# FlagArihant2000/sfm-mvs

Hardware: AMD Instinct MI355X
Metric: descriptor-pair distances/sec (BF-KNN k=2 + Lowe ratio) (higher is better)
Workload: dtype f32 results (bit-identical to the direct-form f32 reference); filter arithmetic on MFMA: i8 MFMA on the descriptors QUANTISED to 8 bits (one grid per pair; the certificate uses the measured residua...; 1 GPU; BASELINE configs[1]: 10k x 10k uniform[0,1) float32 128-D descriptors, BF-KNN k=2 + Lowe ratio 0.70; a step = one launch set = a batch of 8 distinct pairs of that shape per GPU (8e8 distances; 8 distinct pairs per launch set, 2 sets of images rotating over the steps); nq=10000, nt=10000, dim=128

## Files before the change

sfm_mvs_amd/csrc/knn.hip:

```cpp
#include "common.h"
#include <cfloat>
#include <climits>
#include <cstdlib>
#include <type_traits>
#include <algorithm>
#include <mutex>
#include <vector>

namespace {

typedef float f32x16 __attribute__((ext_vector_type(16)));
typedef float f32x4 __attribute__((ext_vector_type(4)));
typedef float f32x3 __attribute__((ext_vector_type(3), aligned(4)));
typedef int i32x3 __attribute__((ext_vector_type(3), aligned(4)));

constexpr int kDim = 128;
constexpr int kTileT = 32;


constexpr int kResidentWaves = 4096;
constexpr int kMaxSlots = 258;
constexpr float kInf = __builtin_huge_valf();
constexpr int kSubTilesHost = 64;
constexpr int kI8SubTilesHost = 128;
// ... 1560 lines not shown
#pragma unroll
        for (int g = 0; g < 2; ++g)
            if (qok[g]) {
                const int64_t ob = ((int64_t)(qrow0 + 32 * g) * (2 * smax * nsub) + (int64_t)slot * nsub * 2 + h) * 3;
                for (int e = sub + 1; e < nsub; ++e)
#pragma unroll
                    for (int r = 0; r < 3; ++r) {
                        cand_s[ob + 6 * e + r] = kInf;
                        cand_i[ob + 6 * e + r] = -1;
                    }
            }
        wait_vmcnt<0>();
        u += t_end - t_begin;
    }
}

template <int ABL, int W>
__global__ __launch_bounds__(64 * W, 2) void knn_filter_split2_kernel(
    const unsigned short* __restrict__ qsplit, const float* __restrict__ qnorm, int nq, int nq_pad,
    const unsigned short* __restrict__ tsplit, int nt, int nt_pad, const float* __restrict__ tn, int tiles, int64_t units,
    int smax, int nsub, const int* __restrict__ midflag, const float* __restrict__ bmax, int force_mode,
    float* __restrict__ cand_s, int* __restrict__ cand_i, const int64_t* __restrict__ wg_begin, const int* __restrict__ rb_first,
    int n_rb1, int n_pairs, int64_t s_qsplit, int64_t s_tsplit, int64_t s_qn, int64_t s_tn, int64_t s_cand, int* __restrict__ minfo,
    const float* __restrict__ bmaxerr, long long* __restrict__ trace) {
    extern __shared__ __attribute__((aligned(16))) float smem[];
    if (trace && threadIdx.x == 0) {
        trace[4 * blockIdx.x + 0] = wall_clock64();
        trace[4 * blockIdx.x + 2] = __builtin_amdgcn_s_getreg(0xF804);
        trace[4 * blockIdx.x + 3] = __builtin_amdgcn_s_getreg(0xF814);
        trace[8192 + 4 * blockIdx.x + 2] = clock64();
    }
    const bool need_mid = (force_mode >= 0 ? force_mode : minfo[kMinfoBatchMode]) == kModeSplit;
    if (need_mid)
        filter_split2_body<ABL, W, true>(smem, qsplit, qnorm, nq, nq_pad, tsplit, nt_pad, tn, tiles, units, smax, nsub, cand_s, cand_i, wg_begin, rb_first,
                                         n_rb1, s_qsplit, s_tsplit, s_qn, s_tn, s_cand, trace);
    else
        filter_split2_body<ABL, W, false>(smem, qsplit, qnorm, nq, nq_pad, tsplit, nt_pad, tn, tiles, units, smax, nsub, cand_s, cand_i, wg_begin, rb_first,
                                          n_rb1, s_qsplit, s_tsplit, s_qn, s_tn, s_cand, trace);
    if (trace && threadIdx.x == 0) {
        trace[4 * blockIdx.x + 1] = wall_clock64();
        trace[8192 + 4 * blockIdx.x + 3] = clock64();
    }
}

constexpr int kQ4Rows = 4 * 4 * 32;
constexpr int kQ4Ring = 3;

typedef int i32x4 __attribute__((ext_vector_type(4)));
typedef int i32x2 __attribute__((ext_vector_type(2)));
typedef unsigned u32x2 __attribute__((ext_vector_type(2)));
#define SFM_MFMA_F16(acc, a, b) asm volatile("v_mfma_f32_32x32x16_f16 %0, %1, %2, %0" : "+v"(acc) : "v"(a), "a"(b))
#define SFM_MFMA_BF16(acc, a, b) asm volatile("v_mfma_f32_32x32x16_bf16 %0, %1, %2, %0" : "+v"(acc) : "v"(a), "a"(b))
#define SFM_MFMA_BF16_INIT(acc, a, b) asm volatile("v_mfma_f32_32x32x8_bf16 %0, %1, %2, 0" : "=v"(acc) : "v"(a), "a"(b))
#define SFM_MFMA_BF16_REINIT(acc, a, b) asm volatile("v_mfma_f32_32x32x8_bf16 %0, %1, %2, 0" : "+v"(acc) : "v"(a), "a"(b))
#define SFM_MFMA_F16_C(acc, a, b, c) asm volatile("v_mfma_f32_32x32x16_f16 %0, %1, %2, %3" : "=&v"(acc) : "v"(a), "a"(b), "v"(c))
#define SFM_MFMA_BF16_C(acc, a, b, c) asm volatile("v_mfma_f32_32x32x16_bf16 %0, %1, %2, %3" : "=&v"(acc) : "v"(a), "a"(b), "v"(c))

__device__ __forceinline__ void key_insert_quad(const f32x16& a, int r, int seq , int vmask, int& k0, int& k1, int& k2) {
    const int m = min(min(__float_as_int(a[r]), __float_as_int(a[r + 1])), min(__float_as_int(a[r + 2]), __float_as_int(a[r + 3])));
    int key;
    asm("v_and_or_b32 %0, %1, %2, %3" : "=v"(key) : "v"(m), "v"(vmask), "s"(seq));
    const int lo = min(key, k0);
    const int m1 = max(min(key, k1), min(max(key, k1), k0));
    k2 = max(min(key, k1), min(max(key, k1), k2));
    k1 = m1;
    k0 = lo;
}

__device__ __forceinline__ int key_make(const f32x16& a, int r, int seq , int vmask) {
    const int m = min(min(__float_as_int(a[r]), __float_as_int(a[r + 1])), min(__float_as_int(a[r + 2]), __float_as_int(a[r + 3])));
    int key;
    asm("v_and_or_b32 %0, %1, %2, %3" : "=v"(key) : "v"(m), "v"(vmask), "s"(seq));
    return key;
}
__device__ __forceinline__ void key_put(int key, int& k0, int& k1, int& k2) {
    const int lo = min(key, k0);
    const int m1 = max(min(key, k1), min(max(key, k1), k0));
    k2 = max(min(key, k1), min(max(key, k1), k2));
    k1 = m1;
    k0 = lo;
}

template <bool KMID, int ABL>
__device__ __forceinline__ void filter_q4_body(
    const unsigned char* __restrict__ qfrag, const unsigned char* __restrict__ tfrag, const unsigned char* __restrict__ qhm,
    const unsigned char* __restrict__ thm, int nq, int nq_pad, int tiles, int smax, int nsub, float* __restrict__ cand_s0,
    int* __restrict__ cand_i0, const int64_t* __restrict__ wg_begin, const int* __restrict__ rb_first, int n_rb1, int64_t s_qfrag,
    int64_t s_tfrag, int64_t s_qhm, int64_t s_thm, int64_t s_cand, const int* __restrict__ minfo, const int* __restrict__ wg_sbase) {
    constexpr int NG = KMID ? 2 : 4;
    constexpr int NPASS = KMID ? 2 : 1;
    constexpr int P = NG / 2;
    constexpr int D = KMID ? 2 : kQ4Ring;
    constexpr int NF = KMID ? 16 : 8;
    const int lane = threadIdx.x & 63;
    const int wave = __builtin_amdgcn_readfirstlane(threadIdx.x >> 6);
    const int j = lane & 31, h = lane >> 5;
    const int G = gridDim.x;
    const int bid = (G & 7) == 0 ? (int)(blockIdx.x & 7) * (G >> 3) + (int)(blockIdx.x >> 3) : (int)blockIdx.x;
    const int64_t u_end = wg_begin[bid + 1];
    int64_t u = wg_begin[bid];
    const int voff = lane * 16, voffi = lane * 8;
    const int qtiles = nq_pad >> 5;
    int vmask;
    asm volatile("v_mov_b32 %0, %1" : "=v"(vmask) : "s"(~kKeyMask));

    while (u < u_end) {
        const int rb = __builtin_amdgcn_readfirstlane((int)(u / tiles));
        const int t_begin = __builtin_amdgcn_readfirstlane((int)(u - (int64_t)rb * tiles));
        const int t_end = __builtin_amdgcn_readfirstlane((int)min((int64_t)tiles, t_begin + (u_end - u)));
        const int sbase = __builtin_amdgcn_readfirstlane(u == wg_begin[bid] ? wg_sbase[bid] : 0);
        const int pb = __builtin_amdgcn_readfirstlane(n_rb1 > 0 ? rb / n_rb1 : 0);
        const int rbl = rb - pb * n_rb1;
        float* __restrict__ cand_s = cand_s0 + pb * s_cand;
        int* __restrict__ cand_i = cand_i0 + pb * s_cand;
        const __amdgpu_buffer_rsrc_t trs = __builtin_amdgcn_make_buffer_rsrc((void*)(tfrag + pb * s_tfrag), 0, tiles * kTileFragBytes, 0x00020000);
        const __amdgpu_buffer_rsrc_t qrs = __builtin_amdgcn_make_buffer_rsrc((void*)(qfrag + pb * s_qfrag), 0, qtiles * kTileFragBytes, 0x00020000);
        const __amdgpu_buffer_rsrc_t thrs = __builtin_amdgcn_make_buffer_rsrc((void*)(KMID ? thm + pb * s_thm : tfrag), 0, KMID ? tiles * 16 * kFragBytes : 0, 0x00020000);
        const __amdgpu_buffer_rsrc_t qhrs = __builtin_amdgcn_make_buffer_rsrc((void*)(KMID ? qhm + pb * s_qhm : qfrag), 0, KMID ? qtiles * 16 * kFragBytes : 0, 0x00020000);

#pragma unroll 1
        for (int pass = 0; pass < NPASS; ++pass) {
            const int qg0 = rbl * (kQ4Rows / 32) + wave * 4 + pass * NG;
            const int qrow0 = qg0 * 32 + j;
            bool qok[NG];
#pragma unroll
            for (int g = 0; g < NG; ++g) qok[g] = qrow0 + 32 * g < nq;

            i32x4 fr[D][NF];
            i32x2 fri[D];
            auto load_frag = [&](int s, int f, int tile_, bool live, bool in_loop = false) {
                if ((ABL & 1) && in_loop) return;
                const int tile = (ABL & 4) ? t_begin : live ? tile_ : t_end - 1;
                if (f == NF) {
                    fri[s] = __builtin_amdgcn_raw_buffer_load_b64(trs, voffi, __builtin_amdgcn_readfirstlane(tile * kTileFragBytes + 8 * kFragBytes), 0);
                } else if constexpr (KMID) {
                    fr[s][f] = __builtin_amdgcn_raw_buffer_load_b128(thrs, voff, __builtin_amdgcn_readfirstlane(tile * (16 * kFragBytes) + f * kFragBytes), 0);
                } else {
                    fr[s][f] = __builtin_amdgcn_raw_buffer_load_b128(trs, voff, __builtin_amdgcn_readfirstlane(tile * kTileFragBytes + f * kFragBytes), 0);
                }
            };
#pragma unroll
            for (int d = 0; d < D; ++d) {
                load_frag(d, NF, t_begin + d, t_begin + d < t_end);
#pragma unroll
                for (int f = 0; f < NF; ++f) load_frag(d, f, t_begin + d, t_begin + d < t_end);
            }

            __builtin_amdgcn_sched_barrier(0);
            u32x4 bq[NG][KMID ? 16 : 8];
            u32x2 bi;
            {
                i32x4 tmp[NG][KMID ? 16 : 8];
#pragma unroll
                for (int g = 0; g < NG; ++g) {
#pragma unroll
                    for (int f = 0; f < (KMID ? 16 : 8); ++f)
                        tmp[g][f] = KMID ? __builtin_amdgcn_raw_buffer_load_b128(qhrs, voff, __builtin_amdgcn_readfirstlane((qg0 + g) * (16 * kFragBytes) + f * kFragBytes), 0)
                                         : __builtin_amdgcn_raw_buffer_load_b128(qrs, voff, __builtin_amdgcn_readfirstlane((qg0 + g) * kTileFragBytes + f * kFragBytes), 0);
                }
                const uint2 qm = frag_init_operand(__int_as_float(minfo[kMinfoQmax + pb]), true, h);
                __builtin_amdgcn_sched_barrier(0);
#pragma unroll
                for (int g = 0; g < NG; ++g) {
#pragma unroll
                    for (int f = 0; f < (KMID ? 16 : 8); ++f) asm volatile("" : "=a"(bq[g][f]) : "0"(__builtin_bit_cast(u32x4, tmp[g][f])));
                }
                asm volatile("" : "=a"(bi) : "0"(u32x2{qm.x, qm.y}));
            }
            asm volatile("s_nop 4");

            int k0[NG], k1[NG], k2[NG];
#pragma unroll
            for (int g = 0; g < NG; ++g) k0[g] = k1[g] = k2[g] = kKeyInf;
            int sub = 0, sub_t0 = t_begin;
            auto flush = [&](int sb, int st0) {
                int qr = qrow0;
                asm volatile("" : "+v"(qr));
#pragma unroll
                for (int g = 0; g < NG; ++g) {
                    if (qok[g]) {
                        const int64_t ob = ((int64_t)(qr + 32 * g) * (2 * smax * nsub) + (int64_t)(sbase + sb) * 2 + h) * 3;
                        flush_keys<true>(k0[g], k1[g], k2[g], st0, h, cand_s + ob, cand_i + ob);
                    }
                    k0[g] = k1[g] = k2[g] = kKeyInf;
                }
            };
            f32x16 acc[NG];
#pragma unroll
            for (int g = P; g < NG; ++g)
#pragma unroll
                for (int r = 0; r < 16; ++r) acc[g][r] = kInf;
            f32x16 cinit;
            SFM_MFMA_BF16_INIT(cinit, __builtin_bit_cast(u32x2, fri[0]), bi);
            asm volatile("s_nop 15\n\ts_nop 7" ::: "memory");

            auto tile = [&](int t, auto slot_c) {
                constexpr int S = decltype(slot_c)::value;
                const bool more = t + D < t_end;
                const int seq_prev = __builtin_amdgcn_readfirstlane(max((t - 1) - sub_t0, 0) << 2);
#pragma unroll
                for (int st = 0; st < 8; ++st) {
                    __builtin_amdgcn_sched_barrier(0);
                    const u32x4 a = __builtin_bit_cast(u32x4, fr[S][st]);
                    if constexpr (KMID) {
                        const u32x4 am = __builtin_bit_cast(u32x4, fr[S][8 + st]);
                        if (st == 0) SFM_MFMA_BF16_C(acc[0], a, bq[0][st], cinit);
                        else SFM_MFMA_BF16(acc[0], a, bq[0][st]);
                        SFM_MFMA_BF16(acc[0], a, bq[0][8 + st]);
                        SFM_MFMA_BF16(acc[0], am, bq[0][st]);
                        if (st & 1) key_insert_quad(acc[1], 4 * (st >> 1), seq_prev + (st >> 1), vmask, k0[1], k1[1], k2[1]);
                    } else {
                        const int g = 2 + (st >> 2);
                        if (st == 0) SFM_MFMA_F16_C(acc[0], a, bq[0][st], cinit);
                        else SFM_MFMA_F16(acc[0], a, bq[0][st]);
                        int key = 0;
                        if (!(ABL & 2)) key = key_make(acc[g], 4 * (st & 3), seq_prev + (st & 3), vmask);
                        __builtin_amdgcn_sched_barrier(0);
                        if (st == 0) SFM_MFMA_F16_C(acc[1], a, bq[1][st], cinit);
                        else SFM_MFMA_F16(acc[1], a, bq[1][st]);
                        if (ABL & 2) {
                            if (st == 0) k0[2] = min(k0[2], __float_as_int(acc[2][0]) + __float_as_int(acc[3][5]));
                        } else
                            key_put(key, k0[g], k1[g], k2[g]);
                    }
                    __builtin_amdgcn_sched_barrier(0);
                }
                if (t - sub_t0 == kSubTiles) {
                    flush(sub, sub_t0);
                    ++sub;
                    sub_t0 = t;
                }
                const int seq_cur = __builtin_amdgcn_readfirstlane((t - sub_t0) << 2);
                __builtin_amdgcn_sched_barrier(0);
                load_frag(S, NF, t + D, more, true);
#pragma unroll
                for (int st = 0; st < 8; ++st) {
                    __builtin_amdgcn_sched_barrier(0);
                    const u32x4 a = __builtin_bit_cast(u32x4, fr[S][st]);
                    if constexpr (KMID) {
                        const u32x4 am = __builtin_bit_cast(u32x4, fr[S][8 + st]);
                        if (st == 0) SFM_MFMA_BF16_C(acc[1], a, bq[1][st], cinit);
                        else SFM_MFMA_BF16(acc[1], a, bq[1][st]);
                        SFM_MFMA_BF16(acc[1], a, bq[1][8 + st]);
                        SFM_MFMA_BF16(acc[1], am, bq[1][st]);
                        if (st == 1) SFM_MFMA_BF16_REINIT(cinit, __builtin_bit_cast(u32x2, fri[(S + 1) % D]), bi);
                    } else {
                        const int g = st >> 2;
                        if (st == 0) SFM_MFMA_F16_C(acc[2], a, bq[2][st], cinit);
                        else SFM_MFMA_F16(acc[2], a, bq[2][st]);
                        int key = 0;
                        if (!(ABL & 2)) key = key_make(acc[g], 4 * (st & 3), seq_cur + (st & 3), vmask);
                        __builtin_amdgcn_sched_barrier(0);
                        if (st == 0) SFM_MFMA_F16_C(acc[3], a, bq[3][st], cinit);
                        else SFM_MFMA_F16(acc[3], a, bq[3][st]);
                        if (st == 1) SFM_MFMA_BF16_REINIT(cinit, __builtin_bit_cast(u32x2, fri[(S + 1) % D]), bi);
                        __builtin_amdgcn_sched_barrier(0);
                        load_frag(S, st, t + D, more, true);
                        if (ABL & 2) {
                            if (st == 0) k0[0] = min(k0[0], __float_as_int(acc[0][0]) + __float_as_int(acc[1][5]));
                        } else
                            key_put(key, k0[g], k1[g], k2[g]);
                    }
                    if constexpr (KMID) {
                        __builtin_amdgcn_sched_barrier(0);
                        load_frag(S, st, t + D, more, true);
                        load_frag(S, 8 + st, t + D, more, true);
                        if (st & 1) key_insert_quad(acc[0], 4 * (st >> 1), seq_cur + (st >> 1), vmask, k0[0], k1[0], k2[0]);
                    }
                    __builtin_amdgcn_sched_barrier(0);
                }
            };
            int t = t_begin;
            for (; t + D <= t_end; t += D) {
                tile(t, std::integral_constant<int, 0>{});
                tile(t + 1, std::integral_constant<int, 1>{});
                if constexpr (D > 2) tile(t + 2, std::integral_constant<int, (D > 2 ? 2 : 0)>{});
            }
            if (t < t_end) {
                tile(t, std::integral_constant<int, 0>{});
                if constexpr (D > 2)
                    if (t + 1 < t_end) tile(t + 1, std::integral_constant<int, 1>{});
            }
            asm volatile("s_nop 15\n\ts_nop 15" ::: "memory");
            if (t_end > t_begin) {
                const int seq = __builtin_amdgcn_readfirstlane(((t_end - 1) - sub_t0) << 2);
#pragma unroll
                for (int g = P; g < NG; ++g)
#pragma unroll
                    for (int r = 0; r < 16; r += 4) key_insert_quad(acc[g], r, seq + (r >> 2), vmask, k0[g], k1[g], k2[g]);
            }
            flush(sub, sub_t0);
        }
        u += t_end - t_begin;
    }
}


typedef int i32x16 __attribute__((ext_vector_type(16)));
#define SFM_MFMA_I8(acc, a, b) asm volatile("v_mfma_i32_32x32x32_i8 %0, %1, %2, %0" : "+v"(acc) : "v"(a), "a"(b))
#define SFM_MFMA_I8_C(acc, a, b, c) asm volatile("v_mfma_i32_32x32x32_i8 %0, %1, %2, %3" : "=&v"(acc) : "v"(a), "a"(b), "v"(c))
#define SFM_MFMA_I8_INIT(acc, a, b) asm volatile("v_mfma_i32_32x32x32_i8 %0, %1, %2, 0" : "=v"(acc) : "v"(a), "a"(b))
#define SFM_MFMA_I8_REINIT(acc, a, b) asm volatile("v_mfma_i32_32x32x32_i8 %0, %1, %2, 0" : "+v"(acc) : "v"(a), "a"(b))

__device__ __forceinline__ int key_pack_i8(int m, int seq ) {
    int key;
    asm("v_lshl_or_b32 %0, %1, 8, %2" : "=v"(key) : "v"(m), "s"(seq));
    return key;
}
__device__ __forceinline__ int imin3(int a, int b, int c) { return min(min(a, b), c); }

template <int ABL>
__device__ __forceinline__ void filter_i8_body(
    const unsigned char* __restrict__ qi8, const unsigned char* __restrict__ ti8, int nq, int nq_pad, int nt, int tiles, int nstr ,
    int* __restrict__ keys0, int* __restrict__ sttab0, const int64_t* __restrict__ wg_begin, int n_rb1, int64_t s_qi8, int64_t s_ti8, int64_t s_keys,
    const int* __restrict__ wg_sbase, int G, int sub_tiles ) {
    constexpr int NG = kI8Groups, P = NG / 2, D = 2;
    const int lane = threadIdx.x & 63;
    const int wave = __builtin_amdgcn_readfirstlane(threadIdx.x >> 6);
    const int j = lane & 31, h = lane >> 5;
    const int bid = (G & 7) == 0 ? (int)(blockIdx.x & 7) * (G >> 3) + (int)(blockIdx.x >> 3) : (int)blockIdx.x;
    const int64_t u_end = wg_begin[bid + 1];
    int64_t u = wg_begin[bid];
    auto train_off = [](int l) { return ((l & ~12) | ((l & 4) << 1) | ((l & 8) >> 1)) * 16; };
    const int voff_t = train_off(lane);
    const int qtiles = nq_pad >> 5;

    while (u < u_end) {
        const int rb = __builtin_amdgcn_readfirstlane((int)(u / tiles));
        const int t_begin = __builtin_amdgcn_readfirstlane((int)(u - (int64_t)rb * tiles));
        const int t_end = __builtin_amdgcn_readfirstlane((int)min((int64_t)tiles, t_begin + (u_end - u)));
        const int sbase = __builtin_amdgcn_readfirstlane(u == wg_begin[bid] ? wg_sbase[bid] : 0);
        const int pb = __builtin_amdgcn_readfirstlane(n_rb1 > 0 ? rb / n_rb1 : 0);
        const int rbl = rb - pb * n_rb1;
        int* __restrict__ keys = keys0 + pb * s_keys;
        int* __restrict__ sttab = sttab0 + (int64_t)rb * nstr * 2;
        const __amdgpu_buffer_rsrc_t trs = __builtin_amdgcn_make_buffer_rsrc((void*)(ti8 + pb * s_ti8), 0, tiles * kI8TileBytes, 0x00020000);
        const __amdgpu_buffer_rsrc_t qrs = __builtin_amdgcn_make_buffer_rsrc((void*)(qi8 + pb * s_qi8), 0, qtiles * kI8QTileBytes, 0x00020000);
        const int qg0 = rbl * (kI8Rows / 32) + wave * NG;
        const int qloc0 = wave * NG * 32 + j;

        i32x4 fr[D][5];
        auto load_frag = [&](int s_, int f, int tile_, bool live, bool in_loop = false) {
            if ((ABL & 1) && in_loop) return;
            const int tile = live ? tile_ : t_end - 1;
            fr[s_][f] = __builtin_amdgcn_raw_buffer_load_b128(trs, voff_t, __builtin_amdgcn_readfirstlane(tile * kI8TileBytes + f * 1024), 0);
        };
#pragma unroll
        for (int d = 0; d < D; ++d) {
            load_frag(d, 4, t_begin + d, t_begin + d < t_end);
#pragma unroll
            for (int f = 0; f < 4; ++f) load_frag(d, f, t_begin + d, t_begin + d < t_end);
        }
        __builtin_amdgcn_sched_barrier(0);
        u32x4 bq[NG][4], bi;
        {
            i32x4 tmp[NG][4];
            int voff_q = voff_t;
            asm volatile("" : "+v"(voff_q));
            const int sw = (voff_q ^ (voff_q >> 1)) & 64;
            voff_q ^= sw | (sw << 1);
#pragma unroll
            for (int g = 0; g < NG; ++g)
#pragma unroll
                for (int f = 0; f < 4; ++f)
                    tmp[g][f] = __builtin_amdgcn_raw_buffer_load_b128(qrs, voff_q, __builtin_amdgcn_readfirstlane((qg0 + g) * kI8QTileBytes + f * 1024), 0);
            __builtin_amdgcn_sched_barrier(0);
#pragma unroll
            for (int g = 0; g < NG; ++g)
#pragma unroll
                for (int f = 0; f < 4; ++f) asm volatile("" : "=a"(bq[g][f]) : "0"(__builtin_bit_cast(u32x4, tmp[g][f])));
            asm volatile("" : "=a"(bi) : "0"(u32x4{h ? 0x80808080u : 0x80808001u, 0x80808080u, 0x80808080u, 0x80808080u}));
        }
        asm volatile("s_nop 4");

        int k0[NG], k1[NG], k2[NG];
#pragma unroll
        for (int g = 0; g < NG; ++g) k0[g] = k1[g] = k2[g] = INT_MAX;
        int sub = 0, sub_t0 = t_begin;
        auto flush = [&](int sb, int st0, int st1) {
            int vo = qloc0 * 16 + h * (kI8Rows * 16);
            asm volatile("" : "+v"(vo));
            const __amdgpu_buffer_rsrc_t krs = __builtin_amdgcn_make_buffer_rsrc(
                (void*)(keys + (int64_t)(rbl * nstr + sbase + sb) * (2 * kI8Rows * 4)), 0, 2 * kI8Rows * 16, 0x00020000);
#pragma unroll
            for (int g = 0; g < NG; ++g) {
                __builtin_amdgcn_raw_buffer_store_b128(u32x4{(unsigned)k0[g], (unsigned)k1[g], (unsigned)k2[g], (unsigned)INT_MAX}, krs, vo + 512 * g, 0, 0);
                k0[g] = k1[g] = k2[g] = INT_MAX;
            }
            if (threadIdx.x == 0) {
                sttab[2 * (sbase + sb)] = st0;
                sttab[2 * (sbase + sb) + 1] = st1 - st0;
            }
        };
        i32x16 acc[NG], cinit;
#pragma unroll
        for (int g = P; g < NG; ++g)
#pragma unroll
            for (int r = 0; r < 16; ++r) acc[g][r] = 0x7FFFFF;
        SFM_MFMA_I8_INIT(cinit, __builtin_bit_cast(u32x4, fr[0][4]), bi);
        asm volatile("s_nop 15\n\ts_nop 7" ::: "memory");

        const int nrem = nt & 31;
        auto mask_tail = [&](i32x16& a) {
#pragma unroll
            for (int r = 0; r < 16; ++r) a[r] = 16 * (r >> 3) + 8 * h + (r & 7) >= nrem ? 0x7FFFFF : a[r];
        };
        int m0 = 0, m1 = 0, n0 = 0, n1 = 0, key = 0, key2 = 0;
        auto epi = [&](int piece, i32x16& a, int seq , int& e0, int& e1, int& e2, bool partial) {
            if (ABL & 2) { if (piece == 0) e0 = min(e0, a[0] + a[15]); return; }
            if (piece == 0 && partial) mask_tail(a);
            if (piece == 0) { m0 = imin3(a[0], a[1], a[2]); n0 = imin3(a[8], a[9], a[10]); m1 = imin3(a[3], a[4], a[5]); n1 = imin3(a[11], a[12], a[13]); }
            else if (piece == 1) { m0 = imin3(m0, m1, a[6]); n0 = imin3(n0, n1, a[14]); m0 = min(m0, a[7]); n0 = min(n0, a[15]); }
            else if (piece == 2) { key = key_pack_i8(m0, seq); key2 = key_pack_i8(n0, seq | 1); key_put(key, e0, e1, e2); }
            else key_put(key2, e0, e1, e2);
            if (piece >= 2) asm volatile("" : "+v"(e0), "+v"(e1), "+v"(e2));
        };
        auto tile = [&](int t, auto slot_c, auto flush_c) {
            constexpr int S = decltype(slot_c)::value;
            constexpr int FL = decltype(flush_c)::value;
            const bool more = t + D < t_end;
            const int seq_prev = __builtin_amdgcn_readfirstlane(max((t - 1) - sub_t0, 0) << 1);
            const bool part_cur = nrem != 0 && t + 1 == tiles;
#pragma unroll
            for (int st = 0; st < 4; ++st) {
                const u32x4 a = __builtin_bit_cast(u32x4, fr[S][st]);
#pragma unroll
                for (int g = 0; g < P; ++g) {
                    __builtin_amdgcn_sched_barrier(0);
                    if (st == 0) SFM_MFMA_I8_C(acc[g], a, bq[g][st], cinit);
                    else SFM_MFMA_I8(acc[g], a, bq[g][st]);
                    epi(g, acc[P + st], seq_prev, k0[P + st], k1[P + st], k2[P + st], false);
                    __builtin_amdgcn_sched_barrier(0);
                }
            }
            if (FL == 1 || (FL == 2 && t - sub_t0 == sub_tiles)) {
                flush(sub, sub_t0, t);
                ++sub;
                sub_t0 = t;
            }
            const int seq_cur = __builtin_amdgcn_readfirstlane((t - sub_t0) << 1);
            __builtin_amdgcn_sched_barrier(0);
            load_frag(S, 4, t + D, more, true);
#pragma unroll
            for (int st = 0; st < 4; ++st) {
                const u32x4 a = __builtin_bit_cast(u32x4, fr[S][st]);
#pragma unroll
                for (int g = 0; g < P; ++g) {
                    __builtin_amdgcn_sched_barrier(0);
                    if (st == 0) SFM_MFMA_I8_C(acc[P + g], a, bq[P + g][st], cinit);
                    else SFM_MFMA_I8(acc[P + g], a, bq[P + g][st]);
                    if (st == 1 && g == 1) SFM_MFMA_I8_REINIT(cinit, __builtin_bit_cast(u32x4, fr[(S + 1) % D][4]), bi);
                    epi(g, acc[st], seq_cur, k0[st], k1[st], k2[st], part_cur);
                    __builtin_amdgcn_sched_barrier(0);
                }
                load_frag(S, st, t + D, more, true);
            }
        };
        constexpr std::integral_constant<int, 0> c0{};
        constexpr std::integral_constant<int, 1> c1{};
        constexpr std::integral_constant<int, 2> c2{};
        int t = t_begin;
        for (;;) {
            const int t_stop = __builtin_amdgcn_readfirstlane(min(sub_t0 + sub_tiles, t_end - (D - 1)));
            for (; t < t_stop; t += D) {
                tile(t, c0, c0);
                tile(t + 1, c1, c0);
                asm volatile("; steady round" ::: "memory");
            }
            if (t + D > t_end) break;
            tile(t, c0, c1);
            tile(t + 1, c1, c0);
            asm volatile("; boundary round" ::: "memory");
            t += D;
        }
        if (t < t_end) tile(t, c0, c2);
        asm volatile("s_nop 15\n\ts_nop 15" ::: "memory");
        if (t_end > t_begin) {
            const int seq = __builtin_amdgcn_readfirstlane(((t_end - 1) - sub_t0) << 1);
#pragma unroll
            for (int g = P; g < NG; ++g)
#pragma unroll
                for (int piece = 0; piece < 4; ++piece) epi(piece, acc[g], seq, k0[g], k1[g], k2[g], nrem != 0 && t_end == tiles);
        }
        flush(sub, sub_t0, t_end);
        u += t_end - t_begin;
    }
}

template <int ABL>
__global__ __launch_bounds__(256, 1) void knn_filter_q4_kernel(
    const unsigned char* __restrict__ qfrag, const unsigned char* __restrict__ tfrag, const unsigned char* __restrict__ qhm,
    const unsigned char* __restrict__ thm, int nq, int nq_pad, int tiles, int smax, int nsub, const int* __restrict__ midflag,
    const float* __restrict__ bmax, int force_mode, float* __restrict__ cand_s, int* __restrict__ cand_i,
    const int64_t* __restrict__ wg_begin, const int* __restrict__ rb_first, int n_rb1, int n_pairs, int64_t s_qfrag, int64_t s_tfrag,
    int64_t s_qhm, int64_t s_thm, int64_t s_cand, int* __restrict__ minfo, const float* __restrict__ bmaxerr,
    const int* __restrict__ wg_sbase, long long* __restrict__ trace,
    const unsigned char* __restrict__ qi8, const unsigned char* __restrict__ ti8, int64_t s_qi8, int64_t s_ti8, int* __restrict__ keys8,
    int* __restrict__ sttab8, int64_t s_keys8, int nstr8, const int64_t* __restrict__ wg_begin8, int n_rb1_8, const int* __restrict__ wg_sbase8, int G8,
    int nt8) {
    if (trace && threadIdx.x == 0) {
        trace[4 * blockIdx.x + 0] = wall_clock64();
        trace[4 * blockIdx.x + 2] = __builtin_amdgcn_s_getreg(0xF804);
        trace[4 * blockIdx.x + 3] = __builtin_amdgcn_s_getreg(0xF814);
        trace[8192 + 4 * blockIdx.x + 2] = clock64();
    }
    if (qi8 && minfo[kMinfoI8]) {
        if ((int)blockIdx.x < G8) filter_i8_body<ABL>(qi8, ti8, nq, nq_pad, nt8, tiles, nstr8, keys8, sttab8, wg_begin8, n_rb1_8, s_qi8, s_ti8, s_keys8, wg_sbase8, G8, minfo[kMinfoSub8]);
        if (trace && threadIdx.x == 0) {
            trace[4 * blockIdx.x + 1] = wall_clock64();
            trace[8192 + 4 * blockIdx.x + 3] = clock64();
        }
        return;
    }
    const bool need_mid = (force_mode >= 0 ? force_mode : minfo[kMinfoBatchMode]) == kModeSplit;
    if (need_mid)
        filter_q4_body<true, 0>(qfrag, tfrag, qhm, thm, nq, nq_pad, tiles, smax, nsub, cand_s, cand_i, wg_begin, rb_first, n_rb1, s_qfrag, s_tfrag, s_qhm,
                             s_thm, s_cand, minfo, wg_sbase);
    else
        filter_q4_body<false, ABL>(qfrag, tfrag, qhm, thm, nq, nq_pad, tiles, smax, nsub, cand_s, cand_i, wg_begin, rb_first, n_rb1, s_qfrag, s_tfrag, s_qhm,
                              s_thm, s_cand, minfo, wg_sbase);
    if (trace && threadIdx.x == 0) {
        trace[4 * blockIdx.x + 1] = wall_clock64();
        trace[8192 + 4 * blockIdx.x + 3] = clock64();
    }
}


__device__ __forceinline__ float lane_odd_neighbour(float v) {
    return __int_as_float(__builtin_amdgcn_update_dpp(0, __float_as_int(v), 0xF5 , 0xF, 0xF, false));
}

__device__ __forceinline__ int imed3(int a, int b, int c) { return max(min(a, b), min(max(a, b), c)); }

struct Best2 {
    float d[2];
    int i[2];
};

__device__ __forceinline__ bool key_less(float da, int ia, float db, int ib) {
    return da < db || (da == db && ia < ib);
}

__device__ __forceinline__ void best2_insert(Best2& b, float d, int i) {
    if (key_less(d, i, b.d[0], b.i[0])) {
        b.d[1] = b.d[0]; b.i[1] = b.i[0];
        b.d[0] = d; b.i[0] = i;
    } else if (key_less(d, i, b.d[1], b.i[1])) {
        b.d[1] = d; b.i[1] = i;
    }
}

__device__ __forceinline__ double dsq_upper(float d) { return (double)d * (double)d * (1.0 + 2.384185791015625e-07); }

constexpr float kU = 5.9604645e-8f;
constexpr float kEpsF32 = 600.f * kU;
static_assert(kKeyBits == 8, "kKeyTrunc = 2^(kKeyBits-23)");
constexpr float kKeyTrunc = 3.0517578e-5f * 1.002f;
constexpr float kEpsRound = 200.f * kU;
constexpr float kChainHalf = 256.f * kU, kChainSplit = 640.f * kU;
constexpr float kEpsSplitOp = 2.33e-5f;
constexpr float kEpsHalfOp = 4.8840e-4f;
constexpr float kEpsHalfAbs = 1.3811e-3f;
constexpr int kModeF32 = 3;

__device__ __forceinline__ void best2_insert_unique(Best2& b, float d, int i) {
    if (i == b.i[0] || i == b.i[1]) return;
    best2_insert(b, d, i);
}

template <int M>
__device__ __forceinline__ void best2_exchange_step(Best2& b) {
    Best2 o;
    o.d[0] = lane_xor<M>(b.d[0]); o.i[0] = lane_xor<M>(b.i[0]);
    o.d[1] = lane_xor<M>(b.d[1]); o.i[1] = lane_xor<M>(b.i[1]);
    best2_insert_unique(b, o.d[0], o.i[0]);
    best2_insert_unique(b, o.d[1], o.i[1]);
}

template <int WIDTH>
__device__ __forceinline__ void best2_group_reduce(Best2& b) {
    if constexpr (WIDTH >= 64) best2_exchange_step<32>(b);
    if constexpr (WIDTH >= 32) best2_exchange_step<16>(b);
    if constexpr (WIDTH >= 16) best2_exchange_step<8>(b);
    if constexpr (WIDTH >= 8) best2_exchange_step<4>(b);
    best2_exchange_step<2>(b);
    best2_exchange_step<1>(b);
}

__device__ __forceinline__ float quad_swap(float v) {
    return __int_as_float(__builtin_amdgcn_update_dpp(0, __float_as_int(v), 0x4E , 0xF, 0xF, false));
}

template <int R, bool NULLABLE>
__device__ __forceinline__ void exact_l2sq_quad_rows(const float* __restrict__ qrow , const float* const (&trow)[R], int j,
                                                     float (&out)[R]) {
    float4 t[R][8];
#pragma unroll
    for (int r = 0; r < R; ++r)
#pragma unroll
        for (int n = 0; n < 8; ++n)
            t[r][n] = (!NULLABLE || trow[r]) ? *reinterpret_cast<const float4*>(trow[r] + 16 * n + 4 * j) : make_float4(0.f, 0.f, 0.f, 0.f);
    float4 acc[R];
#pragma unroll
    for (int r = 0; r < R; ++r) acc[r] = make_float4(0.f, 0.f, 0.f, 0.f);
#pragma unroll
    for (int n = 0; n < 8; ++n) {
        const float4 qv = *reinterpret_cast<const float4*>(qrow + 16 * n + 4 * j);
#pragma unroll
        for (int r = 0; r < R; ++r) {
            const f32x2 d0 = f32x2{qv.x, qv.y} - f32x2{t[r][n].x, t[r][n].y}, d1 = f32x2{qv.z, qv.w} - f32x2{t[r][n].z, t[r][n].w};
            const f32x2 x0 = d0 * d0, x1 = d1 * d1;
#pragma unroll
            for (int half = 0; half < 2; ++half) {
                acc[r].x = quad_swap(acc[r].x) + x0.x;
                acc[r].y = quad_swap(acc[r].y) + x0.y;
                acc[r].z = quad_swap(acc[r].z) + x1.x;
                acc[r].w = quad_swap(acc[r].w) + x1.y;
            }
        }
    }
#pragma unroll
    for (int r = 0; r < R; ++r) {
        const float s0 = acc[r].x + lane_odd_neighbour(acc[r].x), s1 = acc[r].y + lane_odd_neighbour(acc[r].y);
        const float s2 = acc[r].z + lane_odd_neighbour(acc[r].z), s3 = acc[r].w + lane_odd_neighbour(acc[r].w);
        out[r] = ((s0 + s1) + s2) + s3;
    }
}

__device__ __forceinline__ void best2_reduce16_from_quad_lane2(Best2& b) {
    auto bc = [](int v) { return __builtin_amdgcn_update_dpp(0, v, 0xAA , 0xF, 0xF, false); };
    b.d[0] = __int_as_float(bc(__float_as_int(b.d[0]))); b.i[0] = bc(b.i[0]);
    b.d[1] = __int_as_float(bc(__float_as_int(b.d[1]))); b.i[1] = bc(b.i[1]);
    best2_exchange_step<8>(b);
    best2_exchange_step<4>(b);
}

constexpr int kRatioBlock = 1024;
constexpr int kRefQ = 16;
constexpr int kQbStride = 144;
static_assert(kRefQ * kQbStride <= kRefQ * 128 * 2, "the byte rows live in the fp16 body's qhalf / qrows arrays");
constexpr int kS1 = 6;
constexpr int kRescanRows = 1;
constexpr int kRefItems = 512;
constexpr int kPreRows = 2;
constexpr int kHotPre = 2;
constexpr int kRecCap = 112;
constexpr int kQualCap = 144;


struct Best2I {
    float d[2];
    int i[2];
    int s[2];
};
__device__ __forceinline__ void best2i_insert_unique(Best2I& b, float d, int i, int s) {
    if (i == b.i[0] || i == b.i[1]) return;
    if (key_less(d, i, b.d[0], b.i[0])) {
        b.d[1] = b.d[0]; b.i[1] = b.i[0]; b.s[1] = b.s[0];
        b.d[0] = d; b.i[0] = i; b.s[0] = s;
    } else if (key_less(d, i, b.d[1], b.i[1])) {
        b.d[1] = d; b.i[1] = i; b.s[1] = s;
    }
}
template <int M>
__device__ __forceinline__ void best2i_exchange_step(Best2I& b) {
    const float d0 = lane_xor<M>(b.d[0]), d1 = lane_xor<M>(b.d[1]);
    const int i0 = lane_xor<M>(b.i[0]), i1 = lane_xor<M>(b.i[1]), s0 = lane_xor<M>(b.s[0]), s1 = lane_xor<M>(b.s[1]);
    best2i_insert_unique(b, d0, i0, s0);
    best2i_insert_unique(b, d1, i1, s1);
}
constexpr int kRecCapI8 = 56;
constexpr int kS1P = kS1 / 3;
static_assert(kS1 % 3 == 0, "whole pairs");
__device__ __forceinline__ int key_slot(const int* __restrict__ kq, int c) { return kq[(int64_t)(c / 3) * (kI8Rows * 4) + (c % 3)]; }


__device__ __forceinline__ void refine_i8_body(
    const BatchPtrs& P, int B, int nq, int nt, int tiles, const int* __restrict__ minfo, const unsigned char* __restrict__ qi8, const unsigned char* __restrict__ ti8,
    int64_t s_qi8, int64_t s_ti8, const int* __restrict__ wq, const int* __restrict__ wt, int64_t s_qn, int64_t s_tn, const int* __restrict__ keys,
    const int* __restrict__ sttab, int64_t s_keys, int nstr, const int* __restrict__ rb_last8, int n_rb1, int G8, double ratio,
    int* __restrict__ ratio_counts, int ratio_stride, unsigned char* __restrict__ qb , int* __restrict__ recl ,
    int* __restrict__ scratch ) {
    const int n_wg = (nq + kRefQ - 1) / kRefQ, n_tot = B * n_wg, wg_chunk = (n_tot + 7) >> 3;
    const int bidt = n_tot >= 64 ? (int)(blockIdx.x & 7) * wg_chunk + (int)(blockIdx.x >> 3) : (int)blockIdx.x;
    if (bidt >= n_tot) return;
    const int pb = bidt / n_wg, bid = bidt - pb * n_wg;
    const int lane = threadIdx.x & 63, wave = threadIdx.x >> 6;
    const int sub = lane >> 4, sl = lane & 15;
    const int ql = wave * 4 + sub;
    const int q = bid * kRefQ + ql;
    const bool valid = q < nq;
    const int qc = valid ? q : 0;
    const int rbl = (bid * kRefQ) / kI8Rows, rb = pb * n_rb1 + rbl;
    const int qloc = qc - rbl * kI8Rows;
    const int NP = rb_last8[B * n_rb1 + rb] * 2, NC = 3 * NP;
    const int base = minfo[kMinfoBase + pb];
    qi8 += pb * s_qi8; ti8 += pb * s_ti8; wq += pb * s_qn; wt += pb * s_tn; keys += pb * s_keys;
    const int* __restrict__ kq = keys + ((int64_t)rbl * nstr * 2 * kI8Rows + qloc) * 4;
    const int* __restrict__ stt = sttab + (int64_t)rb * nstr * 2;
    int* __restrict__ stats = P.stats[pb];
#ifdef SFM_DEBUG_NREC
    if (bid == 0 && threadIdx.x == 0 && stats) { stats[3] = 4; }
#else
    if (bid == 0 && threadIdx.x == 0 && stats) { stats[1] = G8; stats[2] = 2 * nstr; stats[3] = 4; }
#endif

    if (sl < 8) *reinterpret_cast<uint4*>(qb + ql * kQbStride + 16 * sl) =
        *reinterpret_cast<const uint4*>(qi8 + (int64_t)(qc >> 5) * kI8QTileBytes + (sl >> 1) * 1024 + (((sl & 1) * 32 + (qc & 31)) << 4));
    const int cq = wq[qc] - 128;
    int kv[kS1];
#pragma unroll
    for (int m = 0; m < kS1P; ++m) {
        const int pp = sl + 16 * m;
        const int4 x = (valid && pp < NP) ? *reinterpret_cast<const int4*>(kq + (int64_t)pp * (kI8Rows * 4)) : make_int4(INT_MAX, INT_MAX, INT_MAX, INT_MAX);
        kv[3 * m] = x.x; kv[3 * m + 1] = x.y; kv[3 * m + 2] = x.z;
    }
    auto slot_of = [&](int k) { return 3 * (sl + 16 * (k / 3)) + k % 3; };
    int a1 = INT_MAX, a2 = INT_MAX, atau = INT_MAX;
#pragma unroll
    for (int k = 0; k < kS1; ++k) {
        a2 = imed3(a1, a2, kv[k]);
        a1 = min(a1, kv[k]);
        if (k % 3 == 2) atau = min(atau, kv[k]);
    }
    if (valid)
        for (int pp = sl + 16 * kS1P; pp < NP; pp += 16) {
            const int4 x = *reinterpret_cast<const int4*>(kq + (int64_t)pp * (kI8Rows * 4));
            atau = min(atau, x.z);
            a2 = imed3(a1, a2, x.x); a1 = min(a1, x.x);
            a2 = imed3(a1, a2, x.y); a1 = min(a1, x.y);
            a2 = imed3(a1, a2, x.z); a1 = min(a1, x.z);
        }
    auto fold = [&](int o1, int o2, int ot) {
        const int hi = max(a1, o1);
        a1 = min(a1, o1);
        a2 = min(hi, min(a2, o2));
        atau = min(atau, ot);
    };
    fold(lane_xor<8>(a1), lane_xor<8>(a2), lane_xor<8>(atau));
    fold(lane_xor<4>(a1), lane_xor<4>(a2), lane_xor<4>(atau));
    fold(lane_xor<2>(a1), lane_xor<2>(a2), lane_xor<2>(atau));
    fold(lane_xor<1>(a1), lane_xor<1>(a2), lane_xor<1>(atau));
    const int thr = a2 >= kKeyEmptyI ? kKeyEmptyI - 1 : (int)((((unsigned)(a2 >> 8) + 1u) << 8) | 0xFFu);

    Best2I b;
    b.d[0] = b.d[1] = kInf; b.i[0] = b.i[1] = INT_MAX; b.s[0] = b.s[1] = INT_MAX;
    __builtin_amdgcn_fence(__ATOMIC_RELEASE, "wavefront");
    __builtin_amdgcn_wave_barrier();
    auto eval_row = [&](int tile, int hh, int e, bool live, int qslot, int cqv, Best2I& acc2) {
        const int r = sl & 7;
        const int jr = 16 * e + 8 * hh + r;
        const int row = tile * kTileT + jr;
        const unsigned char* tp = ti8 + (int64_t)tile * kI8TileBytes + (jr << 4);
        uint4 tv[8];
#pragma unroll
        for (int c = 0; c < 8; ++c) tv[c] = *reinterpret_cast<const uint4*>(tp + (c >> 1) * 1024 + (c & 1) * 512);
        const int w = wt[row];
        int s0 = 0, s1 = 0;
#pragma unroll
        for (int c = 0; c < 8; ++c) {
            const uint4 qv = *reinterpret_cast<const uint4*>(qb + qslot * kQbStride + 16 * c);
            s0 = __builtin_amdgcn_sdot4((int)tv[c].x, (int)qv.x, s0, false);
            s1 = __builtin_amdgcn_sdot4((int)tv[c].y, (int)qv.y, s1, false);
            s0 = __builtin_amdgcn_sdot4((int)tv[c].z, (int)qv.z, s0, false);
            s1 = __builtin_amdgcn_sdot4((int)tv[c].w, (int)qv.w, s1, false);
        }
        const int d2 = cqv + w + 2 * (s0 + s1);
        if (live && row < nt) best2i_insert_unique(acc2, sqrtf((float)d2), row, d2);
    };
    auto row_scan = [&](int v, int& total) {
        v += __builtin_amdgcn_update_dpp(0, v, 0x111 , 0xF, 0xF, true);
        v += __builtin_amdgcn_update_dpp(0, v, 0x112 , 0xF, 0xF, true);
        v += __builtin_amdgcn_update_dpp(0, v, 0x114 , 0xF, 0xF, true);
        v += __builtin_amdgcn_update_dpp(0, v, 0x118 , 0xF, 0xF, true);
        total = __builtin_amdgcn_ds_swizzle(v, 0x10 | (0x0F << 5));
        return v;
    };
    auto wave_max = [&](int v) {
        v = max(v, lane_xor<16>(v));
        return max(v, __shfl_xor(v, 32, 64));
    };
    int* __restrict__ myrec = recl + ql * (2 * kRecCapI8);
    int nrec = 0;
    auto process = [&]() {
        __builtin_amdgcn_fence(__ATOMIC_RELEASE, "wavefront");
// ... 1687 lines not shown
```

Measured before the change: 5130 billion distances/s.

## Restructure i8 filter tile loop: scalar load offsets, precomputed seqs, rebalanced epilogue

Reworks the i8 MFMA filter inner loop. Prefetch addresses are now carried as running scalar offsets clamped to the last tile, which drops the per-tile `more` predicate. Sequence keys are precomputed into SGPR state, and the partial-tail masking is moved out of the steady-state path into a dedicated tail tile variant. The epilogue pieces are redistributed so one runs next to the cinit re-init MFMA, and key packing becomes plain C so the compiler can schedule it. The goal is to cut scalar/VALU overhead between MFMAs so the matrix pipe stays busier, at the cost of more complex control flow and bookkeeping for the tail and sub-block boundaries.

```diff
diff --git a/sfm_mvs_amd/csrc/knn.hip b/sfm_mvs_amd/csrc/knn.hip
--- a/sfm_mvs_amd/csrc/knn.hip
+++ b/sfm_mvs_amd/csrc/knn.hip
@@ -1886,11 +1886,7 @@
 #define SFM_MFMA_I8_INIT(acc, a, b) asm volatile("v_mfma_i32_32x32x32_i8 %0, %1, %2, 0" : "=v"(acc) : "v"(a), "a"(b))
 #define SFM_MFMA_I8_REINIT(acc, a, b) asm volatile("v_mfma_i32_32x32x32_i8 %0, %1, %2, 0" : "+v"(acc) : "v"(a), "a"(b))
 
-__device__ __forceinline__ int key_pack_i8(int m, int seq ) {
-    int key;
-    asm("v_lshl_or_b32 %0, %1, 8, %2" : "=v"(key) : "v"(m), "s"(seq));
-    return key;
-}
+__device__ __forceinline__ int key_pack_i8(int m, int seq ) { return (m << 8) | seq; }
 __device__ __forceinline__ int imin3(int a, int b, int c) { return min(min(a, b), c); }
 
 template <int ABL>
@@ -1990,21 +1986,30 @@
             for (int r = 0; r < 16; ++r) a[r] = 16 * (r >> 3) + 8 * h + (r & 7) >= nrem ? 0x7FFFFF : a[r];
         };
         int m0 = 0, m1 = 0, n0 = 0, n1 = 0, key = 0, key2 = 0;
-        auto epi = [&](int piece, i32x16& a, int seq , int& e0, int& e1, int& e2, bool partial) {
+        auto epi = [&](int piece, i32x16& a, int seq , int seq1, int& e0, int& e1, int& e2, bool partial) {
             if (ABL & 2) { if (piece == 0) e0 = min(e0, a[0] + a[15]); return; }
             if (piece == 0 && partial) mask_tail(a);
             if (piece == 0) { m0 = imin3(a[0], a[1], a[2]); n0 = imin3(a[8], a[9], a[10]); m1 = imin3(a[3], a[4], a[5]); n1 = imin3(a[11], a[12], a[13]); }
             else if (piece == 1) { m0 = imin3(m0, m1, a[6]); n0 = imin3(n0, n1, a[14]); m0 = min(m0, a[7]); n0 = min(n0, a[15]); }
-            else if (piece == 2) { key = key_pack_i8(m0, seq); key2 = key_pack_i8(n0, seq | 1); key_put(key, e0, e1, e2); }
-            else key_put(key2, e0, e1, e2);
-            if (piece >= 2) asm volatile("" : "+v"(e0), "+v"(e1), "+v"(e2));
+            else if (piece == 2) { key = key_pack_i8(m0, seq); key_put(key, e0, e1, e2); }
+            else { key2 = key_pack_i8(n0, seq1); key_put(key2, e0, e1, e2); }
+            if (piece >= 2) asm volatile("" :: "v"(e0), "v"(e1), "v"(e2));
         };
-        auto tile = [&](int t, auto slot_c, auto flush_c) {
+        const int ld_last = __builtin_amdgcn_readfirstlane((t_end - 1) * kI8TileBytes);
+        int ld_off = __builtin_amdgcn_readfirstlane(min(t_begin + D - 1, t_end - 1) * kI8TileBytes);
+        int sq = 0, sq1 = 1, sq_n = 0;
+        auto load_next = [&](int s_, int f, int off, int off4) {
+            if (ABL & 1) return;
+            if (f < 4) fr[s_][f] = __builtin_amdgcn_raw_buffer_load_b128(trs, voff_t + f * 1024, off, 0);
+            else fr[s_][f] = __builtin_amdgcn_raw_buffer_load_b128(trs, voff_t, off4, 0);
+        };
+        auto tile = [&](int t, auto slot_c, auto flush_c, auto tail_c) {
             constexpr int S = decltype(slot_c)::value;
             constexpr int FL = decltype(flush_c)::value;
-            const bool more = t + D < t_end;
-            const int seq_prev = __builtin_amdgcn_readfirstlane(max((t - 1) - sub_t0, 0) << 1);
-            const bool part_cur = nrem != 0 && t + 1 == tiles;
+            constexpr int TL = decltype(tail_c)::value;
+            const int seq_prev = sq, seq_prev1 = sq1;
+            const bool part_cur = TL == 2 && nrem != 0 && t + 1 == tiles;
+            int off4 = 0;
 #pragma unroll
             for (int st = 0; st < 4; ++st) {
                 const u32x4 a = __builtin_bit_cast(u32x4, fr[S][st]);
@@ -2013,18 +2018,31 @@
                     __builtin_amdgcn_sched_barrier(0);
                     if (st == 0) SFM_MFMA_I8_C(acc[g], a, bq[g][st], cinit);
                     else SFM_MFMA_I8(acc[g], a, bq[g][st]);
-                    epi(g, acc[P + st], seq_prev, k0[P + st], k1[P + st], k2[P + st], false);
+                    epi(g, acc[P + st], seq_prev, seq_prev1, k0[P + st], k1[P + st], k2[P + st], false);
+                    if (st == 0 && g == 1) ld_off = __builtin_amdgcn_readfirstlane(min(ld_off + kI8TileBytes, ld_last));
+                    if (st == 1 && g == 1) off4 = __builtin_amdgcn_readfirstlane(ld_off + 4 * 1024);
+                    if (st == 2 && g == 1 && FL == 0) { sq = sq_n; sq1 = __builtin_amdgcn_readfirstlane(sq_n | 1); }
                     __builtin_amdgcn_sched_barrier(0);
                 }
             }
-            if (FL == 1 || (FL == 2 && t - sub_t0 == sub_tiles)) {
-                flush(sub, sub_t0, t);
-                ++sub;
-                sub_t0 = t;
-            }
-            const int seq_cur = __builtin_amdgcn_readfirstlane((t - sub_t0) << 1);
+            if (FL != 0) {
+                if (FL == 1 || t - sub_t0 == sub_tiles) {
+                    flush(sub, sub_t0, t);
+                    ++sub;
+                    sub_t0 = t;
+                    sq_n = 0;
+                }
+                sq = sq_n;
+                sq1 = __builtin_amdgcn_readfirstlane(sq_n | 1);
+            }
+            const int seq_cur = sq, seq_cur1 = sq1;
             __builtin_amdgcn_sched_barrier(0);
-            load_frag(S, 4, t + D, more, true);
+            load_next(S, 4, ld_off, off4);
+            int n = 0;
+            auto piece_b = [&]() {
+                if (n < 16) epi(n & 3, acc[n >> 2], seq_cur, seq_cur1, k0[n >> 2], k1[n >> 2], k2[n >> 2], part_cur);
+                ++n;
+            };
 #pragma unroll
             for (int st = 0; st < 4; ++st) {
                 const u32x4 a = __builtin_bit_cast(u32x4, fr[S][st]);
@@ -2033,38 +2051,48 @@
                     __builtin_amdgcn_sched_barrier(0);
                     if (st == 0) SFM_MFMA_I8_C(acc[P + g], a, bq[P + g][st], cinit);
                     else SFM_MFMA_I8(acc[P + g], a, bq[P + g][st]);
-                    if (st == 1 && g == 1) SFM_MFMA_I8_REINIT(cinit, __builtin_bit_cast(u32x4, fr[(S + 1) % D][4]), bi);
-                    epi(g, acc[st], seq_cur, k0[st], k1[st], k2[st], part_cur);
+                    piece_b();
+                    if (st == 1 && g == 1) {
+                        __builtin_amdgcn_sched_barrier(0);
+                        SFM_MFMA_I8_REINIT(cinit, __builtin_bit_cast(u32x4, fr[(S + 1) % D][4]), bi);
+                        __builtin_amdgcn_sched_barrier(0);
+                        piece_b();
+                    }
+                    if (st == 2 && g == 1) sq_n = __builtin_amdgcn_readfirstlane(sq_n + 2);
                     __builtin_amdgcn_sched_barrier(0);
                 }
-                load_frag(S, st, t + D, more, true);
+                load_next(S, st, ld_off, off4);
             }
         };
         constexpr std::integral_constant<int, 0> c0{};
         constexpr std::integral_constant<int, 1> c1{};
         constexpr std::integral_constant<int, 2> c2{};
+        const int t_lim = __builtin_amdgcn_readfirstlane(t_end - (nrem != 0 && t_end == tiles ? 1 : 0));
         int t = t_begin;
         for (;;) {
-            const int t_stop = __builtin_amdgcn_readfirstlane(min(sub_t0 + sub_tiles, t_end - (D - 1)));
+            const int t_stop = __builtin_amdgcn_readfirstlane(min(sub_t0 + sub_tiles, t_lim - (D - 1)));
             for (; t < t_stop; t += D) {
-                tile(t, c0, c0);
-                tile(t + 1, c1, c0);
+                tile(t, c0, c0, c0);
+                tile(t + 1, c1, c0, c0);
                 asm volatile("; steady round" ::: "memory");
             }
-            if (t + D > t_end) break;
-            tile(t, c0, c1);
-            tile(t + 1, c1, c0);
+            if (t + D > t_lim) break;
+            tile(t, c0, c1, c0);
+            tile(t + 1, c1, c0, c0);
             asm volatile("; boundary round" ::: "memory");
             t += D;
         }
-        if (t < t_end) tile(t, c0, c2);
+        if (t < t_end) {
+            tile(t, c0, c2, c2);
+            if (t + 1 < t_end) tile(t + 1, c1, c0, c2);
+        }
         asm volatile("s_nop 15\n\ts_nop 15" ::: "memory");
         if (t_end > t_begin) {
             const int seq = __builtin_amdgcn_readfirstlane(((t_end - 1) - sub_t0) << 1);
 #pragma unroll
             for (int g = P; g < NG; ++g)
 #pragma unroll
-                for (int piece = 0; piece < 4; ++piece) epi(piece, acc[g], seq, k0[g], k1[g], k2[g], nrem != 0 && t_end == tiles);
+                for (int piece = 0; piece < 4; ++piece) epi(piece, acc[g], seq, seq | 1, k0[g], k1[g], k2[g], nrem != 0 && t_end == tiles);
         }
         flush(sub, sub_t0, t_end);
         u += t_end - t_begin;
```

Result: faster. 5202 billion distances/s, median of 6 (+1.4%).
